# LSaldyt/JAX_llama

Hardware: AMD Instinct MI355X
Metric: output_tokens_per_sec (higher is better)
Workload: dtype bf16; 1 GPU; model=llama3-8b, global_batch=2048, seq_len=384, prompt_len=128, gen_len=256, parallelism=dp1, mp=1

## Files before the change

jax_llama_amd/csrc/bindings.cpp:

```cpp
#include <torch/extension.h>
#include <c10/hip/HIPStream.h>

#include "kernels/launchers.h"

#define MODE_RESIDUAL_ID 1
#define MODE_QKV_ID 3
#define MODE_TPRESID_ID 9
#define MODE_ARGMAX_ID 8

namespace {

using torch::Tensor;

hipStream_t stream() { return c10::hip::getCurrentHIPStream().stream(); }

void check(bool cond, const char* msg) { TORCH_CHECK(cond, "jax_llama_amd._C: ", msg); }

void check_gpu(const Tensor& t, const char* name) {
  TORCH_CHECK(t.is_cuda(), "jax_llama_amd._C: ", name, " must be a GPU tensor");
  TORCH_CHECK(t.is_contiguous(), "jax_llama_amd._C: ", name, " must be contiguous");
}

void rc(int r, const char* what) {
  TORCH_CHECK(r == 0, "jax_llama_amd._C: ", what, " failed (code ", r, ")");
// ... 314 lines not shown
                          packed_ptr(out_pack, m, h * dh, "out_pack"), ptr<int32_t>(kv_start), ptr<float>(ws),
                          ptr<int32_t>(tickets), ptr<int32_t>(sync), (int)t_cap, (int)splits, (int)spl, stream(),
                          o_w.has_value() ? o_w->data_ptr() : nullptr, oh, (int)o_n, (int)o_k, o_mode,
                          o_w.has_value() ? &qo : nullptr),
     "linear_qkv_attn");
}

void check_gemm_ws(const c10::optional<Tensor>& ws, int64_t ksplit, int64_t m, int64_t n, bool rms = false) {
  if (ksplit <= 1) return;
  check(ws.has_value(), "gemm: split-K needs a workspace");
  check_gpu(*ws, "gemm ws");
  check(ws->scalar_type() == torch::kFloat32 && ws->numel() >= ksplit * m * (n + (rms ? 1 : 0)),
        "gemm ws too small");
}

void check_g5_ws(const c10::optional<Tensor>& ws, int64_t k, int64_t ksplit, int64_t m, int64_t n, bool rms) {
  check(ws.has_value(), "gemm tile 11 / 12: the slab workspace is required (any split)");
  check_gpu(*ws, "gemm ws");
  const int64_t eks = jla::gemm5_ksplit((int)k, (int)ksplit);
  check(ws->scalar_type() == torch::kFloat32 && ws->numel() >= eks * m * (n + (rms ? 1 : 0)), "gemm ws too small");
}

static float* rms_ws_ptr(const c10::optional<Tensor>& rws, int64_t m, size_t* floats) {
  *floats = 0;
  if (!rws.has_value()) return nullptr;
  check_gpu(*rws, "rms_ws");
  check(rws->scalar_type() == torch::kFloat32 && rws->numel() >= m, "rms_ws: fp32, >= M floats");
  *floats = rws->numel();
  return ptr<float>(*rws);
}

void gemm(Tensor x, Tensor w, int64_t n, int64_t k, Tensor out, int64_t mode, bool accumulate,
          c10::optional<Tensor> mirror, int64_t ksplit, c10::optional<Tensor> ws, double rms_eps, int64_t tile,
          c10::optional<Tensor> pack_out, c10::optional<Tensor> rms_ws) {
  check_gpu(x, "x");
  check_packed(w, n, k);
  check(x.dim() == 2 && x.size(1) == k && x.scalar_type() == torch::kBFloat16, "x must be bf16 [M, K]");
  check(mode >= 0 && mode <= 2, "gemm mode");
  check(rms_eps < 0 || mode != 1, "gemm: fused RMS is not available in residual mode");
  const int64_t m = x.size(0);
  check_linear_out(out, m, n, mode);
  jla::bf16_t* mir = mode == 1 ? mirror_ptr(mirror, out.numel()) : nullptr;
  jla::QKVArgs pqa{};
  if (pack_out.has_value()) {
    check(m <= SKINNY_MAX_M && (mode == 1 || mode == 2) && (mode != 1 || mir), "gemm pack_out: decode M, residual "
          "(with its mirror) or SwiGLU");
    check(ksplit > 1 || tile == 11 || tile == 12, "gemm pack_out: the split-K reduce-kernel path only");
    pqa.pack = packed_ptr(pack_out, m, mode == 2 ? n / 2 : n, "pack_out");
  }
  if (tile == 11 || tile == 12) {
    check_g5_ws(ws, k, ksplit, m, n, rms_eps >= 0);
    rc(jla::gemm(cbf(x), w.data_ptr(), out.data_ptr(), m, n, k, mode, accumulate,
                 out.scalar_type() == torch::kFloat32, mir, pqa.pack ? &pqa : nullptr, ptr<float>(*ws), ws->numel(),
                 ksplit, stream(), (float)rms_eps, (int)tile, nullptr, 0),
       "gemm");
    return;
  }
  check_gemm_ws(ws, ksplit, m, n, rms_eps >= 0);
  size_t rfl = 0;
  float* rws = rms_ws_ptr(rms_ws, m, &rfl);
  rc(jla::gemm(cbf(x), w.data_ptr(), out.data_ptr(), m, n, k, mode, accumulate,
               out.scalar_type() == torch::kFloat32, mir, pqa.pack ? &pqa : nullptr,
               ksplit > 1 ? ptr<float>(*ws) : nullptr, ksplit > 1 ? ws->numel() : 0, ksplit, stream(),
               (float)rms_eps, (int)tile, rws, rfl),
     "gemm");
}

void gemm_qkv(Tensor x, Tensor w, int64_t n, int64_t k, Tensor table, Tensor positions, Tensor kc, Tensor vc,
              Tensor slot, int64_t seq_len, int64_t h, int64_t hkv, int64_t dh, Tensor q, int64_t ksplit,
              c10::optional<Tensor> ws, double rms_eps, int64_t tile, c10::optional<Tensor> rms_ws) {
  check_gpu(x, "x");
  check_packed(w, n, k);
  check(x.dim() == 2 && x.size(1) == k && x.scalar_type() == torch::kBFloat16, "x must be bf16 [M, K]");
  const int64_t m = x.size(0);
  jla::QKVArgs qa = qkv_args(m, n, table, positions, kc, vc, slot, seq_len, h, hkv, dh, q);
  if (tile == 11 || tile == 12) {
    check_g5_ws(ws, k, ksplit, m, n, rms_eps >= 0);
    rc(jla::gemm(cbf(x), w.data_ptr(), nullptr, m, n, k, MODE_QKV_ID, 0, 0, nullptr, &qa, ptr<float>(*ws), ws->numel(),
                 ksplit, stream(), (float)rms_eps, (int)tile, nullptr, 0),
       "gemm_qkv");
    return;
  }
  if (ksplit <= 1) {
    check(rms_eps >= 0 && jla::gemm_qkv_direct_ok((int)m, (int)tile, (int)k), "gemm_qkv without a K split: 256 x 256 FA "
          "tiles with the fused norm (gemm_qkv_direct_ok)");
    size_t rfl = 0;
    float* rws = rms_ws_ptr(rms_ws, m, &rfl);
    rc(jla::gemm(cbf(x), w.data_ptr(), nullptr, m, n, k, MODE_QKV_ID, 0, 0, nullptr, &qa, nullptr, 0, 1, stream(),
                 (float)rms_eps, (int)tile, rws, rfl),
       "gemm_qkv");
    return;
  }
  check(ws.has_value(), "gemm_qkv: a K split needs the slab workspace");
  check_gemm_ws(ws, ksplit, m, n, rms_eps >= 0);
  rc(jla::gemm(cbf(x), w.data_ptr(), nullptr, m, n, k, MODE_QKV_ID, 0, 0, nullptr, &qa, ptr<float>(*ws), ws->numel(),
               ksplit, stream(), (float)rms_eps, (int)tile),
     "gemm_qkv");
// ... 292 lines not shown
    check(out_v->scalar_type() == torch::kFloat32 && out_v->numel() == out_i.numel(), "out_v");
    ov = ptr<float>(*out_v);
  }
  if (mode == 0) {
    check(out_i.numel() == n, "car_pairs argmax out shape");
  } else {
    check(mode == 1 && ov && k > 0 && n % k == 0 && out_i.numel() == n * jla::car_world(st), "car_pairs top-k shapes");
  }
  rc(jla::car_pairs(st, (int)mode, ptr<float>(vals), ptr<int32_t>(idx), (int)idx_offset, n, (int)k, ov,
                    ptr<int32_t>(out_i), stream()),
     "car_pairs");
}

}

PYBIND11_MODULE(TORCH_EXTENSION_NAME, m) {
  m.doc() = "jax_llama_amd gfx950 (MI355X) HIP kernels";
  m.attr("SKINNY_MAX_M") = SKINNY_MAX_M;
  m.attr("ARCH") = "gfx950";
  m.def("embedding", &embedding, py::arg("ids"), py::arg("table"), py::arg("out"),
        py::arg("mirror") = py::none());
  m.def("rms_scale", &rms_scale);
  m.def("rmsnorm", &rmsnorm);
  m.def("residual_add", &residual_add);
  m.def("gemm_f32", &gemm_f32);
  m.def("prefetch", &prefetch, py::arg("t"), py::arg("grid") = 128);
  m.def("linear_skinny", &linear_skinny, py::arg("x"), py::arg("w"), py::arg("n"), py::arg("k"), py::arg("out"),
        py::arg("mode"), py::arg("rms_eps"), py::arg("accumulate"), py::arg("variant"), py::arg("ws"),
        py::arg("tickets"), py::arg("mirror") = py::none(), py::arg("x_packed") = py::none(),
        py::arg("pack_out") = py::none());
  m.def("gemm", &gemm, py::arg("x"), py::arg("w"), py::arg("n"), py::arg("k"), py::arg("out"), py::arg("mode"),
        py::arg("accumulate"), py::arg("mirror") = py::none(), py::arg("ksplit") = 1, py::arg("ws") = py::none(),
        py::arg("rms_eps") = -1.0, py::arg("tile") = 0, py::arg("pack_out") = py::none(),
        py::arg("rms_ws") = py::none());
  m.def("gemm_qkv_direct_ok", [](int64_t m, int64_t tile, int64_t k) {
    return jla::gemm_qkv_direct_ok((int)m, (int)tile, (int)k) != 0;
  });
  m.def("gemm_set_g4_default", [](int64_t on) { jla::gemm_set_g4_default((int)on); });
  m.def("gemm_set_g4_group", [](int64_t gm) { jla::gemm_set_g4_group((int)gm); });
  m.def("gemm_qkv", &gemm_qkv, py::arg("x"), py::arg("w"), py::arg("n"), py::arg("k"), py::arg("table"),
        py::arg("positions"), py::arg("kc"), py::arg("vc"), py::arg("slot"), py::arg("seq_len"), py::arg("h"),
        py::arg("hkv"), py::arg("dh"), py::arg("q"), py::arg("ksplit"), py::arg("ws"), py::arg("rms_eps") = -1.0,
        py::arg("tile") = 0, py::arg("rms_ws") = py::none());
  m.def("gemm_argmax", &gemm_argmax, py::arg("x"), py::arg("w"), py::arg("n"), py::arg("k"), py::arg("ws"),
        py::arg("rms_eps"), py::arg("idx"), py::arg("val"), py::arg("rms_ws") = py::none());
  m.def("gemm_argmax_workspace", [](int64_t m, int64_t n) { return (int64_t)jla::gemm_argmax_workspace_floats(m, n); });
  m.def("gemm_ksplit", [](int64_t m, int64_t n, int64_t k) { return jla::gemm_ksplit(m, n, k); });
  m.def("rope_kv_write", &rope_kv_write);
  m.def("attn_set_impl", [](int64_t impl, int64_t waves_target) { jla::attn_set_impl(impl, waves_target); },
        py::arg("impl"), py::arg("waves_target") = 0);
  m.def("attn_decode_splits",
        [](int64_t b, int64_t hkv, int64_t t, int64_t rep) { return jla::attn_decode_splits(b, hkv, t, rep); });
  m.def("linear_qkv", &linear_qkv, py::arg("x"), py::arg("w"), py::arg("n"), py::arg("k"), py::arg("rms_eps"),
        py::arg("table"), py::arg("positions"), py::arg("kc"), py::arg("vc"), py::arg("slot"), py::arg("seq_len"),
        py::arg("h"), py::arg("hkv"), py::arg("dh"), py::arg("q"), py::arg("variant"), py::arg("ws"), py::arg("tickets"),
        py::arg("x_packed") = py::none());
  m.def("linear_qkv_attn", &linear_qkv_attn, py::arg("x"), py::arg("w"), py::arg("n"), py::arg("k"),
        py::arg("rms_eps"), py::arg("table"), py::arg("positions"), py::arg("kc"), py::arg("vc"), py::arg("slot"),
        py::arg("h"), py::arg("hkv"), py::arg("dh"), py::arg("q"), py::arg("kv_start"), py::arg("out"),
        py::arg("out_pack"), py::arg("ws"), py::arg("tickets"), py::arg("sync"), py::arg("t_cap"), py::arg("splits"),
        py::arg("x_packed") = py::none(), py::arg("spl") = 1, py::arg("sk_ws") = py::none(),
        py::arg("sk_tk") = py::none(), py::arg("o_w") = py::none(), py::arg("o_n") = 0, py::arg("o_k") = 0,
        py::arg("o_h") = py::none(), py::arg("o_hb") = py::none(), py::arg("o_hb_pack") = py::none(),
        py::arg("tp_state") = 0);
  m.def("qkv_attn_splits", [](int64_t m, int64_t b, int64_t hkv, int64_t rep, int64_t t_cap, int64_t n, int64_t cus,
                              int64_t spl, int64_t o_groups) {
    return jla::qkv_attn_splits((int)m, (int)b, (int)hkv, (int)rep, (int)t_cap, (int)n, (int)cus, (int)spl,
// ... 109 lines not shown
```

jax_llama_amd/csrc/kernels/gemm.hip:

```cpp
#include <type_traits>

#include "car.h"
#include "common.h"
#include "gemm4w.h"
#include "gemm5ws.h"
#include "launchers.h"
#include "ring.h"

namespace jla {

constexpr int MODE_PARTIAL = 7;

constexpr int G2_BN = 256, G2_NBUF = 4, G2_DIST = 3, G2_GROUP_M = 8;
#ifdef JLA_GEMM_STAMPS
__device__ unsigned long long g_gemm_stamps[8192 * 8 * 6];
#endif

JLA_DEV void g2_tile_coords(int pid, int tiles_m, int tiles_n, int& tm, int& tn) {
  const int in_group = G2_GROUP_M * tiles_n;
  const int first_m = (pid / in_group) * G2_GROUP_M;
  const int gsz = min(tiles_m - first_m, G2_GROUP_M);
  tm = first_m + (pid % in_group) % gsz;
  tn = (pid % in_group) / gsz;
}
// ... 866 lines not shown
template <int MODE, int RMSM>
__global__ void __launch_bounds__(256, 1)
    gemm4p_kernel(const bf16_t* __restrict__ x, const u32x4* __restrict__ W, void* __restrict__ out, int M, int N,
                  int K, int accumulate, int out_f32, bf16_t* __restrict__ mirror, int tiles_m, int tiles_n,
                  float rms_eps, QKVArgs qa, const float* __restrict__ rms_inv, int group_m) {
  constexpr bool RMS = RMSM == 1;
  __shared__ u32x4 lds[2 * G4_SLOT_U4 + 64];
  const int lane0 = threadIdx.x & 63;
  const int wu = __builtin_amdgcn_readfirstlane(threadIdx.x >> 6);
  const int nwg = gridDim.x, orig = blockIdx.x;
  const int xcd = orig & 7, q8 = nwg >> 3, r8 = nwg & 7;
  const int wg = (xcd < r8 ? xcd * (q8 + 1) : r8 * (q8 + 1) + (xcd - r8) * q8) + (orig >> 3);
  const int tiles = tiles_m * tiles_n;
  const G4Args g{x, W, out, M, N, K, K >> 6, tiles_m, tiles_n};
  const G4Epi ep{out, M, N, K, accumulate, out_f32, mirror, tiles_n, rms_eps, nullptr, rms_inv};
  for (int pid = wg; pid < tiles; pid += nwg) {
    int tm, tn;
    g4_tile_coords(pid, tiles_m, tiles_n, tm, tn, group_m);
    const int m0 = tm * G4_BM, n0 = tn * G4_BN;
    int lane;
    asm volatile("v_mov_b32 %0, %1" : "=v"(lane) : "v"(lane0));
    f32x4 acc[8][8];
#pragma unroll
    for (int j = 0; j < 8; ++j)
#pragma unroll
      for (int i = 0; i < 8; ++i) acc[j][i] = f32x4{0.f, 0.f, 0.f, 0.f};
    float ss[4] = {0.f, 0.f, 0.f, 0.f};
    g4_mainloop<RMS>(g, lds, m0, n0, 0, K >> 6, wu, lane, acc, ss);
    g4_epilogue<MODE, RMSM>(acc, ss, lds, wu, lane, m0, n0, 0, ep, qa);
    __syncthreads();
  }
}

__device__ __forceinline__ float4 sum_splits(const float* __restrict__ ws, int ksplit, size_t slab4, size_t e4) {
  const float4* p = reinterpret_cast<const float4*>(ws) + e4;
  float4 v = p[0];
  for (int s0 = 1; s0 < ksplit; s0 += 8) {
    float4 q[8];
#pragma unroll
    for (int j = 0; j < 8; ++j)
      if (s0 + j < ksplit) q[j] = p[(size_t)(s0 + j) * slab4];
#pragma unroll
    for (int j = 0; j < 8; ++j)
      if (s0 + j < ksplit) {
        v.x += q[j].x;
        v.y += q[j].y;
        v.z += q[j].z;
        v.w += q[j].w;
      }
  }
  return v;
}

template <int MODE>
__global__ void __launch_bounds__(256)
    gemm_reduce_kernel(const float* __restrict__ ws, int ksplit, void* __restrict__ out, int M, int N,
                       int accumulate, int out_f32, bf16_t* __restrict__ mirror, QKVArgs qa,
                       const float* __restrict__ ssq, int K, float rms_eps) {
  const size_t t4 = (size_t)blockIdx.x * blockDim.x + threadIdx.x;
  const size_t slab4 = (size_t)M * N / 4;
  if (t4 >= (MODE == MODE_SWIGLU ? slab4 >> 1 : slab4)) return;
  size_t e4 = t4;
  if constexpr (MODE == MODE_SWIGLU) {
    const size_t oq = (size_t)N >> 3, mo = t4 / oq, c = (t4 - mo * oq) * 4;
    e4 = (mo * N + (c >> 4) * 32 + (c & 15)) >> 2;
  }
// ... 142 lines not shown
#pragma unroll
    for (int i = 0; i < 4; ++i) n[i] = hv[j][i] + sm[i];
    *reinterpret_cast<f32x4*>(h + e4 * 4) = n;
    *reinterpret_cast<u32x2*>(hb + e4 * 4) = u32x2{pack2bf(n[0], n[1]), pack2bf(n[2], n[3])};
  }
  if (threadIdx.x == 0) __hip_atomic_store(d.wg_ctr + w, calls, __ATOMIC_RELAXED, __HIP_MEMORY_SCOPE_AGENT);
}
int gemm_tp_groups(int M, int N) { return (int)(((size_t)M * N + TPR_ELEMS - 1) / TPR_ELEMS); }


static int g2_wm(int M) { return M <= 128 ? 1 : 2; }

int gemm_ksplit(int M, int N, int K) {
  const int KS = K >> 5;
  const int bm = 128 * g2_wm(M);
  const int tiles = ((N + G2_BN - 1) / G2_BN) * ((M + bm - 1) / bm);
  int ks = min(256 / tiles, max(1, K / (2 * M)));
  ks = ks < 1 ? 1 : (ks > 16 ? 16 : ks);
  while (ks > 1 && KS / ks < 4) --ks;
  const int kc = (KS + ks - 1) / ks;
  return (KS + kc - 1) / kc;
}

static int num_cus();
size_t gemm_workspace_floats(int M, int N, int K) {
  const int ks = gemm_ksplit(M, N, K);
  return ks > 1 ? (size_t)ks * M * (N + 1) : 0;
}

static int tile_cfg(int tile, int M) { return tile >= 1 && tile <= 3 ? tile : (M <= 128 ? 2 : 1); }
static bool use_g4(int tile, int M, int K);
constexpr int G4N6D_TILE = 16;
constexpr int G4ND_TILE = 17;
int gemm_qkv_direct_ok(int M, int tile, int K) {
  return ((tile == 0 || tile == 1) && tile_cfg(tile, M) == 1) || use_g4(tile, M, K) ||
         (tile == G4N6D_TILE && (K & 63) == 0);
}

constexpr int G4_TILE = 7;
static bool g_g4_default = true;
void gemm_set_g4_default(int on) { g_g4_default = on != 0; }
constexpr int G4P_TILE = 13;
constexpr int G4D_TILE = 14;
static bool use_g4(int tile, int M, int K) {
  return (K & 63) == 0 &&
         (tile == G4_TILE || tile == G4P_TILE || tile == G4D_TILE || (tile == 0 && g_g4_default && M > 128));
}

static int g_g4_group = 0;
void gemm_set_g4_group(int gm) { g_g4_group = gm; }
static int g4_group_m(int tiles_m, int tiles_n, int K) {
  (void)tiles_n, (void)K;
  const int gm = g_g4_group > 0 ? g_g4_group : 4;
  return gm < tiles_m ? gm : tiles_m;
}
static int g_g5_diag = 0;
template <int MODE, int NJ = 8>
static void launch_g4(const bf16_t* x, const u32x4* w, void* out, int M, int N, int K, int accumulate, int out_f32,
                      bf16_t* mirror, int ksplit, float rms_eps, float* ssq, hipStream_t s, const QKVArgs& qa,
                      float* rms_ws = nullptr, bool persistent = false, bool deep = false) {
  const int tm = (M + G4_BM - 1) / G4_BM, tn = (N + 32 * NJ - 1) / (32 * NJ);
  const int KS64 = K >> 6, kc = (KS64 + ksplit - 1) / ksplit;
  const bool rms = MODE != MODE_RESIDUAL && rms_eps >= 0.f;
  const int grid = tm * tn * ksplit;
  const int gm = g4_group_m(tm, tn, K);
  if constexpr (NJ == 8 && MODE != MODE_PARTIAL && MODE != MODE_ARGMAX) {
// ... 26 lines not shown
  }
  if constexpr (MODE == MODE_STORE) {
    if (!rms && (g_g5_diag & 192)) {
      if ((g_g5_diag & 192) == 64)
        gemm4_kernel<MODE, 0, 8, 1><<<grid, 256, 0, s>>>(x, w, out, M, N, K, accumulate, out_f32, mirror, kc, tm, tn,
                                                        rms_eps, ssq, qa, nullptr, gm);
      else if ((g_g5_diag & 192) == 128)
        gemm4_kernel<MODE, 0, 8, 2><<<grid, 256, 0, s>>>(x, w, out, M, N, K, accumulate, out_f32, mirror, kc, tm, tn,
                                                        rms_eps, ssq, qa, nullptr, gm);
      else
        gemm4_kernel<MODE, 0, 8, 3><<<grid, 256, 0, s>>>(x, w, out, M, N, K, accumulate, out_f32, mirror, kc, tm, tn,
                                                        rms_eps, ssq, qa, nullptr, gm);
      return;
    }
  }
#define JLA_G4(R, INV)                                                                                             \
  if (deep)                                                                                                         \
    gemm4_kernel<MODE, R, 8, 0, true><<<grid, 256, 0, s>>>(x, w, out, M, N, K, accumulate, out_f32, mirror, kc, tm, \
                                                           tn, rms_eps, ssq, qa, INV, gm);                          \
  else                                                                                                              \
    gemm4_kernel<MODE, R><<<grid, 256, 0, s>>>(x, w, out, M, N, K, accumulate, out_f32, mirror, kc, tm, tn, rms_eps, \
                                               ssq, qa, INV, gm)
  if (rms && rms_ws != nullptr && ksplit == 1 && MODE != MODE_PARTIAL) {
    if (rms_rowinv(x, rms_ws, M, K, rms_eps, s) != 0) return;
    JLA_G4(2, rms_ws);
  } else if (rms) {
    JLA_G4(1, nullptr);
  } else {
    JLA_G4(0, nullptr);
  }
#undef JLA_G4
}

template <int MODE>
static void launch_g2(const bf16_t* x, const u32x4* w, void* out, int M, int N, int K, int accumulate, int out_f32,
                      bf16_t* mirror, int kc, int ksplit, float rms_eps, float* ssq, int tile, hipStream_t s,
                      const QKVArgs& qa = QKVArgs{}, float* rms_ws = nullptr) {
  if constexpr (MODE != MODE_QKV && MODE != MODE_ARGMAX) {
    if (tile == G4ND_TILE && (K & 63) == 0) {
      launch_g4<MODE, 4>(x, w, out, M, N, K, accumulate, out_f32, mirror, ksplit, rms_eps, ssq, s, qa, rms_ws, false,
                         true);
      return;
    }
  }
  if constexpr (MODE != MODE_ARGMAX) {
    if (tile == G4N6D_TILE && (K & 63) == 0) {
      launch_g4<MODE, 6>(x, w, out, M, N, K, accumulate, out_f32, mirror, ksplit, rms_eps, ssq, s, qa, rms_ws, false,
                         true);
      return;
    }
  }
  if (use_g4(tile, M, K)) {
    const bool persist = tile == G4P_TILE || (MODE == MODE_RESIDUAL && tile == 0 && ksplit == 1 && M >= 4096);
    launch_g4<MODE>(x, w, out, M, N, K, accumulate, out_f32, mirror, ksplit, rms_eps, ssq, s, qa, rms_ws, persist,
                    tile == G4D_TILE);
    return;
  }
  const int cfg = tile_cfg(tile, M);
  const int bm = cfg == 1 ? 256 : 128, bn = cfg == 3 ? 128 : 256;
  const int tm = (M + bm - 1) / bm, tn = (N + bn - 1) / bn;
  const int grid = tm * tn * ksplit;
#define JLA_G2S(WMV, NB, LATE, R, MTV, NTV, SB)                                                             \
  gemm2_kernel<MODE, WMV, NB, LATE, R, MTV, NTV, SB><<<grid, 256 * WMV, 0, s>>>(                            \
      x, w, out, M, N, K, accumulate, out_f32, mirror, kc, tm, tn, rms_eps, ssq, qa)
#define JLA_G2(WMV, NB, LATE, R, MTV, NTV) JLA_G2S(WMV, NB, LATE, R, MTV, NTV, 1)
#define JLA_G2FA(R, FM)                                                                                      \
  gemm2_kernel<MODE, 2, 4, true, R, 8, 4, 1, true, FM><<<grid, 512, 0, s>>>(x, w, out, M, N, K, accumulate,     \
                                                                           out_f32, mirror, kc, tm, tn, rms_eps, ssq, qa)
  if constexpr (MODE == MODE_QKV) {
    JLA_G2FA(true, 2);
  } else {
  const bool rms = MODE != MODE_RESIDUAL && rms_eps >= 0.f;
  if constexpr (MODE != MODE_RESIDUAL) {
    if (rms) {
      if (cfg == 2)
        JLA_G2(1, 4, false, true, 8, 4);
      else if (cfg == 3)
        JLA_G2(2, 4, true, true, 4, 2);
      else
        JLA_G2FA(true, 2);
      return;
    }
  }
  if (cfg == 2)
    JLA_G2(1, 4, false, false, 8, 4);
  else if (cfg == 3)
    JLA_G2(2, 4, true, false, 4, 2);
  else
    JLA_G2FA(false, 2);
  }
#undef JLA_G2FA
#undef JLA_G2
#undef JLA_G2S
}

template <int MODE>
static void launch_tiled(const bf16_t* x, const u32x4* w, void* out, int M, int N, int K, int accumulate,
                         int out_f32, bf16_t* mirror, int kc, int ksplit, float rms_eps, float* ssq, int tile,
                         hipStream_t s, float* rms_ws = nullptr) {
  launch_g2<MODE>(x, w, out, M, N, K, accumulate, out_f32, mirror, kc, ksplit, rms_eps, ssq, tile, s, QKVArgs{},
                  rms_ws);
}

static int g_num_cus = 0;
static int num_cus() {
  if (g_num_cus == 0) {
    int dev = 0;
    hipDeviceProp_t prop;
    if (hipGetDevice(&dev) == hipSuccess && hipGetDeviceProperties(&prop, dev) == hipSuccess)
      g_num_cus = prop.multiProcessorCount;
    if (g_num_cus <= 0) g_num_cus = 256;
  }
  return g_num_cus;
}

static int launch_reduce(const float* ws, int ksplit, void* out, int M, int N, int K, int mode, int accumulate,
                         int out_f32, bf16_t* mirror, const QKVArgs* qkv, const float* ssq, float rms_eps,
                         hipStream_t s) {
  const size_t total4 = (size_t)M * N / (mode == MODE_SWIGLU ? 8 : 4);
  const int rgrid = (int)((total4 + 255) / 256);
  QKVArgs qa{};
  if (qkv) qa = *qkv;
  const float eps = ssq ? rms_eps : 0.f;
  switch (mode) {
    case MODE_STORE:
      gemm_reduce_kernel<MODE_STORE><<<rgrid, 256, 0, s>>>(ws, ksplit, out, M, N, accumulate, out_f32, nullptr, qa,
                                                           ssq, K, eps);
      break;
    case MODE_RESIDUAL:
      gemm_reduce_kernel<MODE_RESIDUAL><<<rgrid, 256, 0, s>>>(ws, ksplit, out, M, N, accumulate, 1, mirror, qa,
                                                              nullptr, K, eps);
      break;
    case MODE_SWIGLU:
      gemm_reduce_kernel<MODE_SWIGLU><<<rgrid, 256, 0, s>>>(ws, ksplit, out, M, N, accumulate, 0, nullptr, qa, ssq,
                                                            K, eps);
      break;
    case MODE_QKV:
      gemm_reduce_kernel<MODE_QKV><<<rgrid, 256, 0, s>>>(ws, ksplit, out, M, N, accumulate, 0, nullptr, qa, ssq, K,
                                                         eps);
      break;
    case MODE_TPRESID:
      if (!qkv || !qa.tp || !mirror || ssq || (N & 3)) return -1;
      gemm_reduce_tp_kernel<<<gemm_tp_groups(M, N), 256, 0, s>>>(ws, ksplit, static_cast<float*>(out), mirror, M, N,
                                                                 static_cast<const CarDevice*>(qa.tp));
      break;
    default: return -1;
  }
// ... 9 lines not shown
  return (KS64 + kc - 1) / kc;
}
static int launch_g5(const bf16_t* x, const u32x4* w, void* out, int M, int N, int K, int mode, int accumulate,
                     int out_f32, bf16_t* mirror, const QKVArgs* qkv, float* ws, size_t ws_floats, int ksplit,
                     float rms_eps, int tile, hipStream_t s) {
  if ((K & 63) || (N & 15) || M <= 0) return -1;
  if (mode == MODE_SWIGLU && (N & 31)) return -1;
  if (mode == MODE_QKV && !qkv) return -1;
  const bool rms = rms_eps >= 0.f && mode != MODE_RESIDUAL;
  const int KS64 = K >> 6;
  ksplit = gemm5_ksplit(K, ksplit);
  const int kc = (KS64 + ksplit - 1) / ksplit;
  const size_t need = (size_t)ksplit * M * N + (rms ? (size_t)ksplit * M : 0);
  if (ws == nullptr || ws_floats < need) return -3;
  float* ssq = rms ? ws + (size_t)ksplit * M * N : nullptr;
  const int mt = M <= 128 ? 8 : 16, rows = 16 * mt;
  const int ntw = tile == G5_TILE ? 4 : 2;
  const int tiles_m = (M + rows - 1) / rows, tiles_n = (N + 64 * ntw - 1) / (64 * ntw);
  const int grid = tiles_m * tiles_n * ksplit;
  if (mt == 8 && ntw == 4)
    gemm5_partial_kernel<8, 4><<<grid, 256, 0, s>>>(x, w, ws, M, N, K, kc, tiles_m, tiles_n, ssq, g_g5_diag);
  else if (mt == 8)
    gemm5_partial_kernel<8, 2><<<grid, 256, 0, s>>>(x, w, ws, M, N, K, kc, tiles_m, tiles_n, ssq, g_g5_diag);
  else if (ntw == 4)
    gemm5_partial_kernel<16, 4><<<grid, 256, 0, s>>>(x, w, ws, M, N, K, kc, tiles_m, tiles_n, ssq, g_g5_diag);
  else
    gemm5_partial_kernel<16, 2><<<grid, 256, 0, s>>>(x, w, ws, M, N, K, kc, tiles_m, tiles_n, ssq, g_g5_diag);
  JLA_CHECK_LAUNCH();
  return launch_reduce(ws, ksplit, out, M, N, K, mode, accumulate, out_f32, mirror, qkv, ssq, rms_eps, s);
}

int gemm(const bf16_t* x, const void* W, void* out, int M, int N, int K, int mode, int accumulate, int out_f32,
         bf16_t* mirror, const QKVArgs* qkv, float* ws, size_t ws_floats, int ksplit, hipStream_t s,
         float rms_eps, int tile, float* rms_ws, size_t rms_ws_floats) {
  if (tile == G5_TILE || tile == G5_TILE + 1) {
    if (mode == MODE_ARGMAX || (rms_eps >= 0.f && (mode == MODE_RESIDUAL || mode == MODE_TPRESID))) return -1;
    return launch_g5(x, static_cast<const u32x4*>(W), out, M, N, K, mode, accumulate, out_f32, mirror, qkv, ws,
                     ws_floats, ksplit, rms_eps, tile, s);
  }
  if (rms_ws != nullptr && rms_ws_floats < (size_t)M) rms_ws = nullptr;
  if (tile == G4ND_TILE &&
      ((K & 63) || (mode == MODE_QKV && ksplit <= 1) || mode == MODE_ARGMAX ||
       (rms_eps >= 0.f && mode != MODE_RESIDUAL && (ksplit > 1 || rms_ws == nullptr))))
    return -1;
  if (M <= 0) return 0;
  if ((N & 15) || (K & 31)) return -1;
  if (mode == MODE_SWIGLU && (N & 31)) return -1;
  const bool rms = rms_eps >= 0.f;
  if (rms && mode == MODE_RESIDUAL) return -5;
  if (mode == MODE_QKV && !qkv) return -1;
  const int KS = K >> 5;
  if (ksplit < 1) ksplit = 1;
  const int kc = (KS + ksplit - 1) / ksplit;
  ksplit = (KS + kc - 1) / kc;
  if (mode == MODE_TPRESID && (ksplit == 1 || rms)) return -1;
  if (mode == MODE_QKV && ksplit == 1 && !(gemm_qkv_direct_ok(M, tile, K) && rms)) return -1;
  if ((tile == G4ND_TILE || tile == G4N6D_TILE) && rms &&
      (ksplit > 1 || rms_ws == nullptr))
    return -6;
  const u32x4* w = static_cast<const u32x4*>(W);
  if (ksplit == 1) {
    switch (mode) {
      case MODE_QKV:
        launch_g2<MODE_QKV>(x, w, nullptr, M, N, K, 0, 0, nullptr, kc, 1, rms_eps, nullptr, tile, s, *qkv, rms_ws);
        break;
      case MODE_STORE:
        launch_tiled<MODE_STORE>(x, w, out, M, N, K, accumulate, out_f32, nullptr, kc, 1, rms_eps, nullptr, tile, s,
                                 rms_ws);
        break;
      case MODE_RESIDUAL:
        launch_tiled<MODE_RESIDUAL>(x, w, out, M, N, K, accumulate, 1, mirror, kc, 1, -1.f, nullptr, tile, s);
        break;
      case MODE_SWIGLU:
        launch_tiled<MODE_SWIGLU>(x, w, out, M, N, K, accumulate, 0, nullptr, kc, 1, rms_eps, nullptr, tile, s,
                                  rms_ws);
        break;
      default: return -1;
    }
    JLA_CHECK_LAUNCH();
    return 0;
  }
  const size_t need = (size_t)ksplit * M * N + (rms ? (size_t)ksplit * M : 0);
  if ((N & 3) || ws == nullptr || ws_floats < need) return -3;
  float* ssq = rms ? ws + (size_t)ksplit * M * N : nullptr;
  launch_tiled<MODE_PARTIAL>(x, w, ws, M, N, K, 0, 1, nullptr, kc, ksplit, rms_eps, ssq, tile, s);
  JLA_CHECK_LAUNCH();
  return launch_reduce(ws, ksplit, out, M, N, K, mode, accumulate, out_f32, mirror, qkv, ssq, rms_eps, s);
}

JLA_DEV void amax_merge(float& bv, int& bi, float ov, int oi) {
  if (ov > bv || (ov == bv && oi < bi)) {
    bv = ov;
    bi = oi;
  }
}

template <int TPR>
__global__ void __launch_bounds__(TPR == 64 ? 256 : TPR)
    argmax_partials_kernel(const float2* __restrict__ part, int P, int M, int32_t* __restrict__ idx,
                           float* __restrict__ val) {
  __shared__ float s_v[16];
  __shared__ int s_i[16];
  const int row = TPR == 64 ? blockIdx.x * 4 + (threadIdx.x >> 6) : blockIdx.x;
  const int t = TPR == 64 ? (threadIdx.x & 63) : threadIdx.x;
  if (row >= M) return;
  const float2* pr = part + (size_t)row * P;
  float bv[4] = {-INFINITY, -INFINITY, -INFINITY, -INFINITY};
  int bi[4] = {0x7fffffff, 0x7fffffff, 0x7fffffff, 0x7fffffff};
// ... 79 lines not shown
```

jax_llama_amd/csrc/kernels/launchers.h:

```cpp
#pragma once
#include <hip/hip_runtime.h>
#include <stdint.h>

#define SKINNY_MAX_M 64

namespace jla {
typedef uint16_t bf16_t;

int embedding(const int32_t* ids, const bf16_t* table, float* out, bf16_t* mirror, int M, int D, int V,
              hipStream_t s);
int rms_scale(const float* x, bf16_t* out, int M, int D, float eps, hipStream_t s);
int rms_scale_bf16(const bf16_t* x, bf16_t* out, int M, int D, float eps, hipStream_t s);
int rms_rowinv(const bf16_t* x, float* inv, int M, int D, float eps, hipStream_t s);
int residual_add(float* h, const void* p, int p_bf16, bf16_t* hb, long long n, hipStream_t s);
int prefetch(const void* p, long long nbytes, int grid, unsigned* sink, hipStream_t s);
int stream_probe(const void* p, long long nbytes, int grid, unsigned* sink, hipStream_t s);
int gemm_f32(const float* x, const float* w, float* y, int M, int N, int K, hipStream_t s);
int rmsnorm(const float* x, const float* w, float* out, int M, int D, float eps, hipStream_t s);

struct QKVArgs {
  const float2* table;
  int table_len;
  const int32_t* positions;
  bf16_t* kc;
// ... 11 lines not shown
constexpr int CAR_WG_COUNTERS = 4096;
constexpr long long TPRES_REGION = 64 * 64 * 4;

int qkv_attn_o_groups(int M, int rep, int N, int K);
size_t qkv_attn_sync_ints();
void qkv_attn_set_o_nt(int nt);
int qkv_attn_splits(int M, int B, int Hkv, int rep, int t_cap, int N, int cus, int spl = 1, int o_groups = 0);
int qkv_attn_occupancy(int M, int rep, int spl = 1, int o_groups = 0);
void qkv_attn_set_stamps(unsigned long long* p);
void qkv_attn_set_diag(int d);
int linear_qkv_attn(const bf16_t* x, const void* W, int M, int N, int K, float rms_eps, const QKVArgs& qa, bool xp,
                    bf16_t* out, bf16_t* out_pack, const int32_t* kv_start, float* ws, int32_t* tickets, int32_t* sync,
                    int t_cap, int splits, int spl, hipStream_t s,
                    const void* o_w = nullptr, float* o_h = nullptr, int o_n = 0, int o_k = 0, int o_mode = 0,
                    const QKVArgs* qo = nullptr);
int linear_skinny(const void* x, int x_is_f32, const void* W, void* out, int M, int N, int K, int mode,
                  float rms_eps, int accumulate, int out_f32, const QKVArgs* qkv, int variant, hipStream_t s);
constexpr int GEMV_SPLIT_MAX_GROUPS = 1024;
size_t gemv_split_workspace_floats(int M, int N);
int gemv_split_tickets(int N);
inline bool gemv_split_variant(int v) { return v == 16 || v == 18 || v == 26; }
inline bool gemv_xp_variant(int v) { return v == 12 || v == 15 || v == 18 || v == 21 || v == 22 || v == 26; }
int gemm_ksplit(int M, int N, int K);
int gemm_qkv_direct_ok(int M, int tile, int K);
void gemm_set_g4_default(int on);
void gemm_set_g4_group(int gm);
int gemm5_ksplit(int K, int ksplit);
int clock_probe(int iters, int grid, unsigned long long* out, hipStream_t s);
void gemm5_set_diag(int d);
size_t gemm_workspace_floats(int M, int N, int K);
int gemm_tp_groups(int M, int N);
int gemm(const bf16_t* x, const void* W, void* out, int M, int N, int K, int mode, int accumulate, int out_f32,
         bf16_t* mirror, const QKVArgs* qkv, float* ws, size_t ws_floats, int ksplit, hipStream_t s,
         float rms_eps = -1.f, int tile = 0, float* rms_ws = nullptr, size_t rms_ws_floats = 0);
int gemm_argmax(const bf16_t* x, const void* W, float* ws, size_t ws_floats, int M, int N, int K, float rms_eps,
                int32_t* idx, float* val, hipStream_t s, float* rms_ws = nullptr, size_t rms_ws_floats = 0);
size_t gemm_argmax_workspace_floats(int M, int N);
int argmax_partials(const float* part, int P, int M, int32_t* idx, float* val, hipStream_t s);

int rope_kv_write(const bf16_t* qkv, const float* table, int table_len, const int32_t* positions, bf16_t* kc,
                  bf16_t* vc, const int32_t* slot, int M, int S, int H, int Hkv, int Dh, int T, bf16_t* q_out,
                  hipStream_t s);

int attn_decode_chunk(int B, int Hkv, int T, int rep);
void attn_set_v5_max_pairs(int n);
void attn_set_v5_fold(int n);
void attn_set_v3_max_pairs(int n);
void attn_set_impl(int impl, int waves_target);
void attn_set_diag(int d);
void attn_set_v3_kpg(int mult);
unsigned jla_bounds_norm_embed(int reset);
unsigned jla_bounds_rope_kv(int reset);
unsigned jla_bounds_sample(int reset);
unsigned jla_bounds_gemm(int reset);
unsigned jla_bounds_gemv(int reset);
unsigned jla_bounds_attn_decode(int reset);
unsigned jla_bounds_attn_prefill(int reset);
int attn_decode_splits(int B, int Hkv, int T, int rep);
int attn_decode(const bf16_t* q, const bf16_t* kc, const bf16_t* vc, const int32_t* slot, const int32_t* kv_start,
                const uint8_t* key_mask, int mask_len, bf16_t* out, float* ws, int32_t* tickets, int B, int H,
                int Hkv, int Dh, int T, int t_cap, int nsplit, hipStream_t s, bf16_t* out_pack = nullptr);
int attn_decode_packs(int B, int Hkv, int rep);
int attn_decode_v6(const bf16_t* q, const bf16_t* kc, const bf16_t* vc, const int32_t* slot, const int32_t* kv_start,
                   const uint8_t* key_mask, int mask_len, bf16_t* out, int B, int H, int Hkv, int T, int t_cap,
                   hipStream_t s, bf16_t* out_pack);
void attn_set_v6(int mode);
void attn_set_v6_wpp(int wpp);
// ... 39 lines not shown
```

jax_llama_amd/ops/autotune.py:

```python
from __future__ import annotations

import contextlib
import json
import os
from typing import Dict, Optional, Tuple

import torch

_CACHE: Dict[Tuple, int] = {}
ENABLED = os.environ.get("JLA_AUTOTUNE", "1") != "0"
ARCH = "gfx950"

_SCOPE = {"comm": None}


@contextlib.contextmanager
def tp_scope(comm):
    prev = _SCOPE["comm"]
    _SCOPE["comm"] = comm if comm is not None and getattr(comm, "size", 1) > 1 else None
    try:
        yield
    finally:
        _SCOPE["comm"] = prev


def _collective(decide):
    comm = _SCOPE["comm"]
    if comm is None or comm.group is None and not _dist_ready():
        return decide()
    import torch.distributed as dist
    obj = [decide() if comm.rank == 0 else None]
    src = dist.get_global_rank(comm.group, 0) if comm.group is not None else 0
    dist.broadcast_object_list(obj, src=src, group=comm.group)
    v = obj[0]
    return tuple(v) if isinstance(v, list) else v


def _dist_ready() -> bool:
    import torch.distributed as dist
    return dist.is_available() and dist.is_initialized()


_LOADED = {"done": False}


def tune_file() -> str:
    env = os.environ.get("JLA_TUNE_FILE")
    if env:
        return env
    base = os.environ.get("XDG_CACHE_HOME") or os.path.join(os.path.expanduser("~"), ".cache")
    return os.path.join(base, "jax_llama_amd", f"tune_{ARCH}.json")


TUNE_VERSION = 12


def _key_str(kind: str, key: Tuple) -> str:
    return f"{kind}@{TUNE_VERSION}:" + ",".join(str(k).replace("torch.", "") for k in key)


PACKAGED_FILE = os.path.join(os.path.dirname(os.path.abspath(__file__)), f"tune_{ARCH}.json")


def _read_table(path: str) -> Dict[str, object]:
    try:
        with open(path) as f:
            data = json.load(f)
    except (OSError, ValueError):
        return {}
    return data if isinstance(data, dict) else {}


def _load():
    if _LOADED["done"]:
        return
    _LOADED["done"] = True
    if not _persist_on():
        return
    if os.environ.get("JLA_TUNE_PACKAGED", "1") != "0":
        _PERSISTED.update(_read_table(PACKAGED_FILE))
    _PERSISTED.update(_read_table(tune_file()))


_PERSISTED: Dict[str, object] = {}


def _persist_on() -> bool:
# ... 120 lines not shown
            graphs[v] = None
    ev0, ev1 = torch.cuda.Event(enable_timing=True), torch.cuda.Event(enable_timing=True)
    times = {v: float("inf") for v in cands}
    for _ in range(TUNE_ROUNDS):
        for v in cands:
            g = graphs[v]
            ev0.record()
            if g is not None:
                g.replay()
            else:
                for i in range(iters):
                    run(v, x, ws[i % copies])
            ev1.record()
            ev1.synchronize()
            times[v] = min(times[v], ev0.elapsed_time(ev1) / iters)
    del ws, graphs
    _TIMES[(x.shape[0], w.n, w.k, len(_TIMES))] = {v: round(t * 1000.0, 2) for v, t in times.items()}
    return min(cands, key=times.get)


_TIMES: Dict[Tuple, Dict[int, float]] = {}


def table() -> Dict[Tuple, int]:
    return dict(_CACHE)


def measured() -> Dict[Tuple, Dict[int, float]]:
    return dict(_TIMES)


_KS_CACHE: Dict[Tuple, Tuple[int, int]] = {}
KS_CANDIDATES = (1, 2, 3, 4, 6, 8, 12, 16)
TILE_CANDIDATES = (1, 2, 3, 7, 11, 12, 14, 16, 17)
if os.environ.get("JLA_TUNE_TILES"):
    TILE_CANDIDATES = tuple(int(v) for v in os.environ["JLA_TUNE_TILES"].split(","))
TUNE_MAX_M = int(os.environ.get("JLA_TUNE_MAX_M", "4096"))


def choose_gemm_plan(e, m: int, n: int, k: int, device, mode: int = 0, rms: bool = False) -> Tuple[int, int]:
    mode = 0 if mode == 3 else mode
    key = (m, n, k, mode, bool(rms), _SCOPE["comm"] is not None)
    plan = _KS_CACHE.get(key)
    if plan is not None:
        return plan
    heur = e.gemm_ksplit(m, n, k)
    if m <= 128 or m > TUNE_MAX_M or not ENABLED or device.type != "cuda" or torch.cuda.is_current_stream_capturing():
        return heur, 0
    def decide():
        pv = _persisted("gemm", key[:-1])
        if isinstance(pv, tuple) and len(pv) == 2:
            return pv
        mv = _measure_plan(e, m, n, k, device, heur, mode, rms)
        _save("gemm", key[:-1], mv)
        return mv

    plan = tuple(_collective(decide))
    _KS_CACHE[key] = plan
    return plan


def choose_gemm_ksplit(e, m: int, n: int, k: int, device) -> int:
    return choose_gemm_plan(e, m, n, k, device)[0]


G4N_TILES = (16, 17)
G5_TILES = (11, 12)
TUNE_ROUNDS = 3


TUNE_WS_BYTES = int(float(os.environ.get("JLA_TUNE_WS_GB", "4")) * (1 << 30))


def _measure_plan(e, m, n, k, device, heur, mode=0, rms=False) -> Tuple[int, int]:
    kt = k // 32

    def fits(c):
        return c * m * (n + 1) * 4 <= TUNE_WS_BYTES

    ks_c = sorted({c for c in KS_CANDIDATES if kt // c >= 4 and fits(c)} | ({heur} if fits(heur) else set()) | {1})
    cands = [(c, tm) for tm in TILE_CANDIDATES for c in ks_c
             if (tm not in G4N_TILES or (k % 64 == 0 and not (c > 1 and rms and mode != 1)))
             and (tm not in G5_TILES or (k % 64 == 0 and m <= 512))]
    if k % 64 == 0 and m <= 512:
        cands += [(c, tm) for tm in G5_TILES for c in (24, 32, 48) if (k // 64) // c >= 2 and c not in ks_c and fits(c)]
    nbytes = n * k * 2
    copies = max(2, min(16, (640 << 20) // max(nbytes, 1) + 1))
    ws_w = [torch.empty(n // 16, k // 32, 64, 8, dtype=torch.bfloat16, device=device).normal_(0, 0.02)
            for _ in range(copies)]
    x = torch.randn(m, k, device=device).to(torch.bfloat16)
    mirror = None
    if mode == 1:
        out = torch.zeros(m, n, dtype=torch.float32, device=device)
        mirror = torch.empty(m, n, dtype=torch.bfloat16, device=device)
    else:
        out = torch.empty(m, n // 2 if mode == 2 else n, dtype=torch.bfloat16, device=device)
    eps = 1e-5 if (rms and mode != 1) else -1.0
    need = max(c for c, _ in cands) * m * (n + 1)
    ws = torch.empty(need, dtype=torch.float32, device=device)
    ev0, ev1 = torch.cuda.Event(enable_timing=True), torch.cuda.Event(enable_timing=True)
    rms_ws = torch.empty(m, dtype=torch.float32, device=device)

    def run(c, tm, i):
        if tm in G5_TILES:
            e.gemm(x, ws_w[i % copies], n, k, out, mode, True, mirror, c, ws, eps, tm)
        else:
            e.gemm(x, ws_w[i % copies], n, k, out, mode, True, mirror, c, ws if c > 1 else None, eps, tm,
                   None, rms_ws if c == 1 and eps > 0 else None)

    for c, tm in cands:
        for i in range(2):
            run(c, tm, i)
    times = {cand: float("inf") for cand in cands}
    iters = 2 * copies
    for _ in range(TUNE_ROUNDS):
# ... 20 lines not shown
```

Baseline: 43430 tokens/s.

## Add mixed body/tail GEMM tiles to balance wave quantization across CUs

Adds two new GEMM tile variants (18/19) that cover most columns with wide 256x192 or 256x256 body tiles and the remaining columns with 256x128 tail tiles, all in a single launch. A cost model picks the body/tail split so the number of scheduling rounds across CUs is reduced compared with a uniform grid. The launch also remaps block IDs across XCDs. The autotuner gains these tiles as candidates and its cache version is bumped, so they are used only when measured faster, at the price of longer tuning and more kernel instantiations.

```diff
diff --git a/jax_llama_amd/csrc/bindings.cpp b/jax_llama_amd/csrc/bindings.cpp
--- a/jax_llama_amd/csrc/bindings.cpp
+++ b/jax_llama_amd/csrc/bindings.cpp
@@ -370,9 +370,18 @@
 
 void gemm(Tensor x, Tensor w, int64_t n, int64_t k, Tensor out, int64_t mode, bool accumulate,
           c10::optional<Tensor> mirror, int64_t ksplit, c10::optional<Tensor> ws, double rms_eps, int64_t tile,
-          c10::optional<Tensor> pack_out, c10::optional<Tensor> rms_ws) {
+          c10::optional<Tensor> pack_out, c10::optional<Tensor> rms_ws, int64_t n_body) {
   check_gpu(x, "x");
   check_packed(w, n, k);
+  if (tile == 18 || tile == 19) {
+    const int64_t wb = jla::gemm_tail_width((int)tile);
+    check(ksplit <= 1 && k % 64 == 0, "gemm tiles 18 / 19: no K split, K % 64 == 0");
+    check(n_body >= 0 && n_body * wb < n, "gemm tiles 18 / 19: the body must leave columns for the tail");
+    check(n_body > 0 || jla::gemm_tail_split((int)((x.size(0) + 255) / 256), (int)n, (int)wb, jla::gemm_num_cus()) > 0,
+          "gemm tiles 18 / 19: no tail split beats the uniform grid for this shape (gemm_tail_split)");
+  } else {
+    check(n_body == 0, "gemm n_body: tiles 18 / 19 only");
+  }
   check(x.dim() == 2 && x.size(1) == k && x.scalar_type() == torch::kBFloat16, "x must be bf16 [M, K]");
   check(mode >= 0 && mode <= 2, "gemm mode");
   check(rms_eps < 0 || mode != 1, "gemm: fused RMS is not available in residual mode");
@@ -400,7 +409,7 @@
   rc(jla::gemm(cbf(x), w.data_ptr(), out.data_ptr(), m, n, k, mode, accumulate,
                out.scalar_type() == torch::kFloat32, mir, pqa.pack ? &pqa : nullptr,
                ksplit > 1 ? ptr<float>(*ws) : nullptr, ksplit > 1 ? ws->numel() : 0, ksplit, stream(),
-               (float)rms_eps, (int)tile, rws, rfl),
+               (float)rms_eps, (int)tile, rws, rfl, (int)n_body),
      "gemm");
 }
 
@@ -759,7 +768,11 @@
   m.def("gemm", &gemm, py::arg("x"), py::arg("w"), py::arg("n"), py::arg("k"), py::arg("out"), py::arg("mode"),
         py::arg("accumulate"), py::arg("mirror") = py::none(), py::arg("ksplit") = 1, py::arg("ws") = py::none(),
         py::arg("rms_eps") = -1.0, py::arg("tile") = 0, py::arg("pack_out") = py::none(),
-        py::arg("rms_ws") = py::none());
+        py::arg("rms_ws") = py::none(), py::arg("n_body") = 0);
+  m.def("gemm_tail_split", [](int64_t tiles_m, int64_t n, int64_t width, int64_t cus) {
+    const int nb = jla::gemm_tail_split((int)tiles_m, (int)n, (int)width, cus > 0 ? (int)cus : jla::gemm_num_cus());
+    return std::make_pair((int64_t)nb, nb > 0 ? (n - nb * width + 127) / 128 : (int64_t)0);
+  }, py::arg("tiles_m"), py::arg("n"), py::arg("width"), py::arg("cus") = 0);
   m.def("gemm_qkv_direct_ok", [](int64_t m, int64_t tile, int64_t k) {
     return jla::gemm_qkv_direct_ok((int)m, (int)tile, (int)k) != 0;
   });
diff --git a/jax_llama_amd/csrc/kernels/gemm.hip b/jax_llama_amd/csrc/kernels/gemm.hip
--- a/jax_llama_amd/csrc/kernels/gemm.hip
+++ b/jax_llama_amd/csrc/kernels/gemm.hip
@@ -922,6 +922,51 @@
   }
 }
 
+template <int MODE, int RMSM, int NJ>
+JLA_DEV void g4t_tile(const G4Args& g, const G4Epi& ep, u32x4* lds, int m0, int n0, int wu, int lane) {
+  f32x4 acc[NJ][8];
+#pragma unroll
+  for (int j = 0; j < NJ; ++j)
+#pragma unroll
+    for (int i = 0; i < 8; ++i) acc[j][i] = f32x4{0.f, 0.f, 0.f, 0.f};
+  float ss[4] = {0.f, 0.f, 0.f, 0.f};
+  if constexpr (NJ != 8) {
+    g4n_mainloop<NJ, decltype(acc), true>(g, lds, m0, n0, 0, g.K >> 6, wu, lane, acc);
+  } else {
+    g4_mainloop<false, decltype(acc), 0, true>(g, lds, m0, n0, 0, g.K >> 6, wu, lane, acc, ss);
+  }
+  g4_epilogue<MODE, RMSM, decltype(acc), NJ>(acc, ss, lds, wu, lane, m0, n0, 0, ep, QKVArgs{});
+}
+
+JLA_DEV int g4t_remap(int orig, int nwg) {
+  const int xcd = orig & 7, q8 = nwg >> 3, r8 = nwg & 7;
+  return (xcd < r8 ? xcd * (q8 + 1) : r8 * (q8 + 1) + (xcd - r8) * q8) + (orig >> 3);
+}
+
+template <int MODE, int RMSM, int NJB>
+__global__ void __launch_bounds__(256, 1)
+    gemm4t_kernel(const bf16_t* __restrict__ x, const u32x4* __restrict__ W, void* __restrict__ out, int M, int N,
+                  int K, int accumulate, int out_f32, bf16_t* __restrict__ mirror, int tiles_m, int nb, int nt,
+                  float rms_eps, const float* __restrict__ rms_inv, int group_m) {
+  static_assert(NJB == 6 || NJB == 8, "body tiles: 256 x 192 / 256 x 256");
+  static_assert(RMSM != 1 && MODE != MODE_ARGMAX && MODE != MODE_QKV && MODE != MODE_PARTIAL, "see above");
+  __shared__ u32x4 lds[2 * G4_A_U4 + 3 * G4_B_U4];
+  const int lane = threadIdx.x & 63;
+  const int wu = __builtin_amdgcn_readfirstlane(threadIdx.x >> 6);
+  const int body = tiles_m * nb, orig = blockIdx.x;
+  const G4Epi ep{out, M, N, K, accumulate, out_f32, mirror, 0, rms_eps, nullptr, rms_inv};
+  int tm, tn;
+  if (orig < body) {
+    g4_tile_coords(g4t_remap(orig, body), tiles_m, nb, tm, tn, group_m);
+    const G4Args g{x, W, out, M, N, K, K >> 6, tiles_m, nb};
+    g4t_tile<MODE, RMSM, NJB>(g, ep, lds, tm * G4_BM, tn * (32 * NJB), wu, lane);
+  } else {
+    g4_tile_coords(g4t_remap(orig - body, tiles_m * nt), tiles_m, nt, tm, tn, group_m);
+    const G4Args g{x, W, out, M, N, K, K >> 6, tiles_m, nt};
+    g4t_tile<MODE, RMSM, 4>(g, ep, lds, tm * G4_BM, nb * (32 * NJB) + tn * 128, wu, lane);
+  }
+}
+
 __device__ __forceinline__ float4 sum_splits(const float* __restrict__ ws, int ksplit, size_t slab4, size_t e4) {
   const float4* p = reinterpret_cast<const float4*>(ws) + e4;
   float4 v = p[0];
@@ -1130,6 +1175,28 @@
 static bool use_g4(int tile, int M, int K);
 constexpr int G4N6D_TILE = 16;
 constexpr int G4ND_TILE = 17;
+constexpr int G4T6_TILE = 18;
+constexpr int G4T8_TILE = 19;
+static bool is_g4t(int tile) { return tile == G4T6_TILE || tile == G4T8_TILE; }
+int gemm_tail_width(int tile) { return tile == G4T6_TILE ? 192 : (tile == G4T8_TILE ? 256 : 0); }
+
+int gemm_tail_split(int tiles_m, int N, int width, int cus) {
+  if (tiles_m <= 0 || N <= 0 || cus <= 0 || (width != 192 && width != 256)) return 0;
+  auto rounds = [&](long long wgs) { return (wgs + cus - 1) / cus; };
+  auto tail_tiles = [&](int nb) { return (N - nb * width + 127) / 128; };
+  auto aligned = [&](int nb) { return (tiles_m * nb) % 8 == 0 && (tiles_m * tail_tiles(nb)) % 8 == 0; };
+  long long best = rounds((long long)tiles_m * ((N + width - 1) / width)) * width * 16;
+  int best_nb = 0;
+  for (int nb = (N - 1) / width; nb >= 1; --nb) {
+    const long long cost =
+        rounds((long long)tiles_m * nb) * width * 16 + rounds((long long)tiles_m * tail_tiles(nb)) * 128 * 17;
+    if (cost < best || (best_nb != 0 && cost == best && aligned(nb) && !aligned(best_nb))) {
+      best = cost;
+      best_nb = nb;
+    }
+  }
+  return best_nb;
+}
 int gemm_qkv_direct_ok(int M, int tile, int K) {
   return ((tile == 0 || tile == 1) && tile_cfg(tile, M) == 1) || use_g4(tile, M, K) ||
          (tile == G4N6D_TILE && (K & 63) == 0);
@@ -1222,10 +1289,36 @@
 #undef JLA_G4
 }
 
+template <int MODE, int NJB>
+static void launch_g4t(const bf16_t* x, const u32x4* w, void* out, int M, int N, int K, int accumulate, int out_f32,
+                       bf16_t* mirror, float rms_eps, hipStream_t s, float* rms_ws, int n_body) {
+  const int tm = (M + G4_BM - 1) / G4_BM, nt = (N - n_body * 32 * NJB + 127) / 128;
+  const bool rms = MODE != MODE_RESIDUAL && rms_eps >= 0.f;
+  const int grid = tm * (n_body + nt);
+  const int gm = g4_group_m(tm, n_body, K);
+  if (rms) {
+    if (rms_ws == nullptr || rms_rowinv(x, rms_ws, M, K, rms_eps, s) != 0) return;
+    gemm4t_kernel<MODE, 2, NJB><<<grid, 256, 0, s>>>(x, w, out, M, N, K, accumulate, out_f32, mirror, tm, n_body, nt,
+                                                     rms_eps, rms_ws, gm);
+  } else {
+    gemm4t_kernel<MODE, 0, NJB><<<grid, 256, 0, s>>>(x, w, out, M, N, K, accumulate, out_f32, mirror, tm, n_body, nt,
+                                                     rms_eps, nullptr, gm);
+  }
+}
+
 template <int MODE>
 static void launch_g2(const bf16_t* x, const u32x4* w, void* out, int M, int N, int K, int accumulate, int out_f32,
                       bf16_t* mirror, int kc, int ksplit, float rms_eps, float* ssq, int tile, hipStream_t s,
-                      const QKVArgs& qa = QKVArgs{}, float* rms_ws = nullptr) {
+                      const QKVArgs& qa = QKVArgs{}, float* rms_ws = nullptr, int n_body = 0) {
+  if constexpr (MODE == MODE_STORE || MODE == MODE_RESIDUAL || MODE == MODE_SWIGLU) {
+    if (is_g4t(tile)) {
+      if (tile == G4T6_TILE)
+        launch_g4t<MODE, 6>(x, w, out, M, N, K, accumulate, out_f32, mirror, rms_eps, s, rms_ws, n_body);
+      else
+        launch_g4t<MODE, 8>(x, w, out, M, N, K, accumulate, out_f32, mirror, rms_eps, s, rms_ws, n_body);
+      return;
+    }
+  }
   if constexpr (MODE != MODE_QKV && MODE != MODE_ARGMAX) {
     if (tile == G4ND_TILE && (K & 63) == 0) {
       launch_g4<MODE, 4>(x, w, out, M, N, K, accumulate, out_f32, mirror, ksplit, rms_eps, ssq, s, qa, rms_ws, false,
@@ -1287,9 +1380,9 @@
 template <int MODE>
 static void launch_tiled(const bf16_t* x, const u32x4* w, void* out, int M, int N, int K, int accumulate,
                          int out_f32, bf16_t* mirror, int kc, int ksplit, float rms_eps, float* ssq, int tile,
-                         hipStream_t s, float* rms_ws = nullptr) {
+                         hipStream_t s, float* rms_ws = nullptr, int n_body = 0) {
   launch_g2<MODE>(x, w, out, M, N, K, accumulate, out_f32, mirror, kc, ksplit, rms_eps, ssq, tile, s, QKVArgs{},
-                  rms_ws);
+                  rms_ws, n_body);
 }
 
 static int g_num_cus = 0;
@@ -1303,6 +1396,7 @@
   }
   return g_num_cus;
 }
+int gemm_num_cus() { return num_cus(); }
 
 static int launch_reduce(const float* ws, int ksplit, void* out, int M, int N, int K, int mode, int accumulate,
                          int out_f32, bf16_t* mirror, const QKVArgs* qkv, const float* ssq, float rms_eps,
@@ -1378,7 +1472,7 @@
 
 int gemm(const bf16_t* x, const void* W, void* out, int M, int N, int K, int mode, int accumulate, int out_f32,
          bf16_t* mirror, const QKVArgs* qkv, float* ws, size_t ws_floats, int ksplit, hipStream_t s,
-         float rms_eps, int tile, float* rms_ws, size_t rms_ws_floats) {
+         float rms_eps, int tile, float* rms_ws, size_t rms_ws_floats, int n_body) {
   if (tile == G5_TILE || tile == G5_TILE + 1) {
     if (mode == MODE_ARGMAX || (rms_eps >= 0.f && (mode == MODE_RESIDUAL || mode == MODE_TPRESID))) return -1;
     return launch_g5(x, static_cast<const u32x4*>(W), out, M, N, K, mode, accumulate, out_f32, mirror, qkv, ws,
@@ -1404,6 +1498,13 @@
   if ((tile == G4ND_TILE || tile == G4N6D_TILE) && rms &&
       (ksplit > 1 || rms_ws == nullptr))
     return -6;
+  if (is_g4t(tile)) {
+    if ((K & 63) || ksplit > 1 || (mode != MODE_STORE && mode != MODE_RESIDUAL && mode != MODE_SWIGLU)) return -1;
+    if (rms && rms_ws == nullptr) return -6;
+    const int wb = gemm_tail_width(tile);
+    if (n_body <= 0) n_body = gemm_tail_split((M + G4_BM - 1) / G4_BM, N, wb, num_cus());
+    if (n_body <= 0 || (long long)n_body * wb >= N) return -7;
+  }
   const u32x4* w = static_cast<const u32x4*>(W);
   if (ksplit == 1) {
     switch (mode) {
@@ -1412,14 +1513,15 @@
         break;
       case MODE_STORE:
         launch_tiled<MODE_STORE>(x, w, out, M, N, K, accumulate, out_f32, nullptr, kc, 1, rms_eps, nullptr, tile, s,
-                                 rms_ws);
+                                 rms_ws, n_body);
         break;
       case MODE_RESIDUAL:
-        launch_tiled<MODE_RESIDUAL>(x, w, out, M, N, K, accumulate, 1, mirror, kc, 1, -1.f, nullptr, tile, s);
+        launch_tiled<MODE_RESIDUAL>(x, w, out, M, N, K, accumulate, 1, mirror, kc, 1, -1.f, nullptr, tile, s, nullptr,
+                                    n_body);
         break;
       case MODE_SWIGLU:
         launch_tiled<MODE_SWIGLU>(x, w, out, M, N, K, accumulate, 0, nullptr, kc, 1, rms_eps, nullptr, tile, s,
-                                  rms_ws);
+                                  rms_ws, n_body);
         break;
       default: return -1;
     }
diff --git a/jax_llama_amd/csrc/kernels/launchers.h b/jax_llama_amd/csrc/kernels/launchers.h
--- a/jax_llama_amd/csrc/kernels/launchers.h
+++ b/jax_llama_amd/csrc/kernels/launchers.h
@@ -67,7 +67,10 @@
 int gemm_tp_groups(int M, int N);
 int gemm(const bf16_t* x, const void* W, void* out, int M, int N, int K, int mode, int accumulate, int out_f32,
          bf16_t* mirror, const QKVArgs* qkv, float* ws, size_t ws_floats, int ksplit, hipStream_t s,
-         float rms_eps = -1.f, int tile = 0, float* rms_ws = nullptr, size_t rms_ws_floats = 0);
+         float rms_eps = -1.f, int tile = 0, float* rms_ws = nullptr, size_t rms_ws_floats = 0, int n_body = 0);
+int gemm_tail_width(int tile);
+int gemm_tail_split(int tiles_m, int N, int width, int cus);
+int gemm_num_cus();
 int gemm_argmax(const bf16_t* x, const void* W, float* ws, size_t ws_floats, int M, int N, int K, float rms_eps,
                 int32_t* idx, float* val, hipStream_t s, float* rms_ws = nullptr, size_t rms_ws_floats = 0);
 size_t gemm_argmax_workspace_floats(int M, int N);
diff --git a/jax_llama_amd/ops/autotune.py b/jax_llama_amd/ops/autotune.py
--- a/jax_llama_amd/ops/autotune.py
+++ b/jax_llama_amd/ops/autotune.py
@@ -52,7 +52,7 @@
     return os.path.join(base, "jax_llama_amd", f"tune_{ARCH}.json")
 
 
-TUNE_VERSION = 12
+TUNE_VERSION = 13
 
 
 def _key_str(kind: str, key: Tuple) -> str:
@@ -239,7 +239,7 @@
 
 _KS_CACHE: Dict[Tuple, Tuple[int, int]] = {}
 KS_CANDIDATES = (1, 2, 3, 4, 6, 8, 12, 16)
-TILE_CANDIDATES = (1, 2, 3, 7, 11, 12, 14, 16, 17)
+TILE_CANDIDATES = (1, 2, 3, 7, 11, 12, 14, 16, 17, 18, 19)
 if os.environ.get("JLA_TUNE_TILES"):
     TILE_CANDIDATES = tuple(int(v) for v in os.environ["JLA_TUNE_TILES"].split(","))
 TUNE_MAX_M = int(os.environ.get("JLA_TUNE_MAX_M", "4096"))
@@ -272,6 +272,7 @@
 
 
 G4N_TILES = (16, 17)
+G4T_TILES = {18: 192, 19: 256}
 G5_TILES = (11, 12)
 TUNE_ROUNDS = 3
 
@@ -288,6 +289,8 @@
     ks_c = sorted({c for c in KS_CANDIDATES if kt // c >= 4 and fits(c)} | ({heur} if fits(heur) else set()) | {1})
     cands = [(c, tm) for tm in TILE_CANDIDATES for c in ks_c
              if (tm not in G4N_TILES or (k % 64 == 0 and not (c > 1 and rms and mode != 1)))
+             and (tm not in G4T_TILES or (k % 64 == 0 and c == 1
+                                          and e.gemm_tail_split((m + 255) // 256, n, G4T_TILES[tm])[0] > 0))
              and (tm not in G5_TILES or (k % 64 == 0 and m <= 512))]
     if k % 64 == 0 and m <= 512:
         cands += [(c, tm) for tm in G5_TILES for c in (24, 32, 48) if (k // 64) // c >= 2 and c not in ks_c and fits(c)]
```

New measurement: 44040 tokens/s, median of 6. 1.01x the previous value.
